# radoslawkrolikowski/financial-market-data-analysis

Measured on NVIDIA H100. Metric: sequences/sec (train step) biGRU h=256 seq=128 feat=64, higher is better.
Workload: dtype bf16x3 (fp32-class: split bf16 operand pairs on tensor cores, fp32 accumulate / state / gradients)

## Files before the change

### financial_market_data_analysis_b200/csrc/tc_hopper.cuh

```cuda
#pragma once
#include "common.cuh"
#include "kernels_f32.cuh"
#include <algorithm>
#include <map>
#include <mutex>
#include <cuda.h>
#include <cuda_bf16.h>

namespace htc {

typedef __nv_bfloat16 bf16_t;

__device__ __forceinline__ uint32_t smem_u32(const void* p) { return (uint32_t)__cvta_generic_to_shared(p); }

__device__ __forceinline__ void split_bf16(float x, bf16_t& hi, bf16_t& lo) {
    hi = __float2bfloat16(x);
    lo = __float2bfloat16(x - __bfloat162float(hi));
}

__device__ __forceinline__ void ldsm_x4(uint32_t addr, uint32_t (&r)[4]) {
    asm volatile("ldmatrix.sync.aligned.m8n8.x4.shared.b16 {%0, %1, %2, %3}, [%4];"
                 : "=r"(r[0]), "=r"(r[1]), "=r"(r[2]), "=r"(r[3]) : "r"(addr));
}
__device__ __forceinline__ void ldsm_x2(uint32_t addr, uint32_t (&r)[2]) {
// ... 28 lines not shown
}

constexpr int WG_BM = 128, WG_BN = 128, WG_BK = 64;
constexpr int WG_CBOX = 64 * 32 * 4;
__host__ __device__ constexpr int wg_cboxes(int ns) { return ns == 1 ? 4 : 2; }
__host__ __device__ constexpr int wg_smem_bytes(int ns, int stages) {
    return 1024 + stages * 2 * (ns == 1 ? 1 : 2) * WG_BM * WG_BK * 2 + 2 * wg_cboxes(ns) * WG_CBOX + 2 * stages * 8;
}

__global__ void tc_pack_kernel(const float* __restrict__ src, int64_t s_r, int64_t s_k, int64_t zsrc, int R, int K, int Rp, int Kp,
                               bf16_t* __restrict__ hi, bf16_t* __restrict__ lo) {
    __shared__ float tile[32][33];
    const int z = blockIdx.z, r0 = blockIdx.y * 32, k0 = blockIdx.x * 32;
    const float* a = src + z * zsrc;
    const bool kfast = s_k == 1;
    for (int j = threadIdx.y; j < 32; j += 8) {
        const int r = r0 + (kfast ? j : threadIdx.x), k = k0 + (kfast ? threadIdx.x : j);
        float v = 0.f;
        if (r < R && k < K) v = a[(int64_t)r * s_r + (int64_t)k * s_k];
        if (kfast) tile[j][threadIdx.x] = v; else tile[threadIdx.x][j] = v;
    }
    __syncthreads();
    for (int j = threadIdx.y; j < 32; j += 8) {
        const int r = r0 + j, k = k0 + threadIdx.x;
        const int64_t o = ((int64_t)z * Rp + r) * Kp + k;
        bf16_t h, l;
        split_bf16(tile[j][threadIdx.x], h, l);
        hi[o] = h;
        if (lo) lo[o] = l;
    }
}

__global__ void to_planes_kernel(const float* __restrict__ src, int64_t rows, int cols, int pitch, bf16_t* __restrict__ hi,
                                 bf16_t* __restrict__ lo) {
    const int64_t n = rows * cols;
    for (int64_t i = (int64_t)blockIdx.x * blockDim.x + threadIdx.x; i < n; i += (int64_t)gridDim.x * blockDim.x) {
        const int64_t r = i / cols, c = i % cols, o = r * pitch + c;
        bf16_t h, l;
        split_bf16(src[i], h, l);
        hi[o] = h;
        if (lo) lo[o] = l;
    }
}

__device__ __forceinline__ void mbar_init(uint64_t* bar, uint32_t count) {
    asm volatile("mbarrier.init.shared::cta.b64 [%0], %1;" ::"r"(smem_u32(bar)), "r"(count) : "memory");
}
__device__ __forceinline__ void mbar_arrive_expect_tx(uint64_t* bar, uint32_t bytes) {
    asm volatile("mbarrier.arrive.expect_tx.shared::cta.b64 _, [%0], %1;" ::"r"(smem_u32(bar)), "r"(bytes) : "memory");
}
__device__ __forceinline__ void mbar_arrive(uint64_t* bar) {
    asm volatile("mbarrier.arrive.shared::cta.b64 _, [%0];" ::"r"(smem_u32(bar)) : "memory");
}
__device__ __forceinline__ bool mbar_try_wait(uint64_t* bar, uint32_t parity) {
    uint32_t ok;
    asm volatile(
        "{\n\t.reg .pred p;\n\t"
        "mbarrier.try_wait.parity.shared::cta.b64 p, [%1], %2;\n\t"
        "selp.u32 %0, 1, 0, p;\n\t}" : "=r"(ok) : "r"(smem_u32(bar)), "r"(parity) : "memory");
    return ok != 0;
}
__device__ __forceinline__ bool mbar_try_wait_cluster(uint64_t* bar, uint32_t parity) {
    uint32_t ok;
    asm volatile(
        "{\n\t.reg .pred p;\n\t"
        "mbarrier.try_wait.parity.acquire.cluster.shared::cta.b64 p, [%1], %2;\n\t"
        "selp.u32 %0, 1, 0, p;\n\t}" : "=r"(ok) : "r"(smem_u32(bar)), "r"(parity) : "memory");
    return ok != 0;
}
template <bool CLUSTER = false>
__device__ __forceinline__ void mbar_wait(uint64_t* bar, uint32_t parity) {
    auto ready = [&] { return CLUSTER ? mbar_try_wait_cluster(bar, parity) : mbar_try_wait(bar, parity); };
    if (ready()) return;
    uint64_t t0, t;
    asm volatile("mov.u64 %0, %%globaltimer;" : "=l"(t0));
    for (uint32_t i = 0;; ++i) {
        if (ready()) return;
        if ((i & 1023u) == 1023u) {
            asm volatile("mov.u64 %0, %%globaltimer;" : "=l"(t));
            if (t - t0 > 5000000000ull) __trap();
        }
    }
}
__device__ __forceinline__ void bulk_copy_to_peer(uint32_t src, uint32_t bytes, uint64_t* bar, uint32_t cta) {
    asm volatile("cp.async.bulk.shared::cluster.shared::cta.mbarrier::complete_tx::bytes [%0], [%1], %2, [%3];"
                 ::"r"(mapa(src, cta)), "r"(src), "r"(bytes), "r"(mapa(smem_u32(bar), cta)) : "memory");
}
__device__ __forceinline__ void tma_load_3d(uint32_t dst, const CUtensorMap* m, uint64_t* bar, int c0, int c1, int c2) {
    asm volatile("cp.async.bulk.tensor.3d.shared::cluster.global.mbarrier::complete_tx::bytes [%0], [%1, {%3, %4, %5}], [%2];"
                 ::"r"(dst), "l"(reinterpret_cast<uint64_t>(m)), "r"(smem_u32(bar)), "r"(c0), "r"(c1), "r"(c2) : "memory");
}
__device__ __forceinline__ void tma_store_3d(const CUtensorMap* m, uint32_t src, int c0, int c1, int c2) {
    asm volatile("cp.async.bulk.tensor.3d.global.shared::cta.bulk_group [%0, {%2, %3, %4}], [%1];"
                 ::"l"(reinterpret_cast<uint64_t>(m)), "r"(src), "r"(c0), "r"(c1), "r"(c2) : "memory");
}
__device__ __forceinline__ void bulk_commit() { asm volatile("cp.async.bulk.commit_group;" ::: "memory"); }
template <int N>
__device__ __forceinline__ void bulk_wait_read() { asm volatile("cp.async.bulk.wait_group.read %0;" ::"n"(N) : "memory"); }
__device__ __forceinline__ void bulk_wait_all() { asm volatile("cp.async.bulk.wait_group 0;" ::: "memory"); }
__device__ __forceinline__ void named_sync(int id, int n) { asm volatile("bar.sync %0, %1;" ::"r"(id), "r"(n) : "memory"); }
__device__ __forceinline__ uint64_t wg_desc(uint32_t saddr, uint32_t lbo) {
    return (uint64_t)((saddr & 0x3FFFF) >> 4) | ((uint64_t)(lbo >> 4) << 16) | ((uint64_t)(1024 >> 4) << 32) | ((uint64_t)1 << 62);
}
template <int TA, int TB>
__device__ __forceinline__ void wgmma_m64n128k16(float (&d)[64], uint64_t da, uint64_t db) {
    asm volatile("wgmma.mma_async.sync.aligned.m64n128k16.f32.bf16.bf16 {%0, %1, %2, %3, %4, %5, %6, %7, %8, %9, %10, %11, %12, %13, %14, %15, %16, %17, %18, %19, %20, %21, %22, %23, %24, %25, %26, %27, %28, %29, %30, %31, %32, %33, %34, %35, %36, %37, %38, %39, %40, %41, %42, %43, %44, %45, %46, %47, %48, %49, %50, %51, %52, %53, %54, %55, %56, %57, %58, %59, %60, %61, %62, %63}, %64, %65, 1, 1, 1, %66, %67;"
                 : "+f"(d[0]), "+f"(d[1]), "+f"(d[2]), "+f"(d[3]), "+f"(d[4]), "+f"(d[5]), "+f"(d[6]), "+f"(d[7]), "+f"(d[8]), "+f"(d[9]), "+f"(d[10]), "+f"(d[11]), "+f"(d[12]), "+f"(d[13]), "+f"(d[14]), "+f"(d[15]), "+f"(d[16]), "+f"(d[17]), "+f"(d[18]), "+f"(d[19]), "+f"(d[20]), "+f"(d[21]), "+f"(d[22]), "+f"(d[23]), "+f"(d[24]), "+f"(d[25]), "+f"(d[26]), "+f"(d[27]), "+f"(d[28]), "+f"(d[29]), "+f"(d[30]), "+f"(d[31]), "+f"(d[32]), "+f"(d[33]), "+f"(d[34]), "+f"(d[35]), "+f"(d[36]), "+f"(d[37]), "+f"(d[38]), "+f"(d[39]), "+f"(d[40]), "+f"(d[41]), "+f"(d[42]), "+f"(d[43]), "+f"(d[44]), "+f"(d[45]), "+f"(d[46]), "+f"(d[47]), "+f"(d[48]), "+f"(d[49]), "+f"(d[50]), "+f"(d[51]), "+f"(d[52]), "+f"(d[53]), "+f"(d[54]), "+f"(d[55]), "+f"(d[56]), "+f"(d[57]), "+f"(d[58]), "+f"(d[59]), "+f"(d[60]), "+f"(d[61]), "+f"(d[62]), "+f"(d[63])
                 : "l"(da), "l"(db), "n"(TA), "n"(TB));
}

struct WgOp {
    int zsel, coff, kshift[2];
};
struct WgJob {
    WgOp a, b;
    float* C; const float* bias; float* part;
    int M, N, tm, tn, batch, splits;
    int kblocks, kbd;
    int kcat;
    int beta;
    int cmap;
    int64_t ldc, zC, zBias;
};

template <int NS, int STAGES, int AMN, int BMN>
__global__ void __launch_bounds__(384, 1)
wg_gemm_kernel(const __grid_constant__ CUtensorMap ta_hi, const __grid_constant__ CUtensorMap ta_lo,
               const __grid_constant__ CUtensorMap tb_hi, const __grid_constant__ CUtensorMap tb_lo,
               const __grid_constant__ CUtensorMap tc, const WgJob j) {
    constexpr int NH = NS == 1 ? 1 : 2;
    constexpr int PLANE = WG_BM * WG_BK * 2;
    constexpr int STAGE = 2 * NH * PLANE;
    constexpr int CB = wg_cboxes(NS);
    extern __shared__ __align__(1024) uint8_t wg_smem_raw[];
    uint8_t* sm = reinterpret_cast<uint8_t*>((reinterpret_cast<uintptr_t>(wg_smem_raw) + 1023) & ~(uintptr_t)1023);
    uint64_t* full = reinterpret_cast<uint64_t*>(sm + STAGES * STAGE + 2 * CB * WG_CBOX);
    uint64_t* empty = full + STAGES;
    const int wgi = threadIdx.x / 128, tid = threadIdx.x % 128;
    const int units = j.tm * j.tn * j.batch * j.splits;
    const int per = (j.kblocks + j.splits - 1) / j.splits;
    if (threadIdx.x == 0) {
        for (int i = 0; i < STAGES; ++i) { mbar_init(full + i, 1); mbar_init(empty + i, 2); }
        asm volatile("fence.mbarrier_init.release.cluster;" ::: "memory");
    }
    __syncthreads();
    auto decode = [&](int u, int& s, int& zb, int& m0, int& n0) {
        s = u % j.splits; u /= j.splits;
        n0 = (u % j.tn) * WG_BN; u /= j.tn;
        m0 = (u % j.tm) * WG_BM; zb = u / j.tm;
    };

    if (wgi == 0) {
        if (tid == 0) {
            uint32_t it = 0;
            for (int u = blockIdx.x; u < units; u += gridDim.x) {
                int s, zb, m0, n0;
                decode(u, s, zb, m0, n0);
                const int kb1 = min(j.kblocks, (s + 1) * per);
                for (int kb = s * per; kb < kb1; ++kb, ++it) {
                    const int st = it % STAGES;
                    if (it >= STAGES) mbar_wait(empty + st, ((it / STAGES) - 1) & 1);
                    const uint32_t base = smem_u32(sm + st * STAGE);
                    mbar_arrive_expect_tx(full + st, STAGE);
                    const int dz = j.kcat ? kb / j.kbd : zb, kc = (j.kcat ? kb % j.kbd : kb) * WG_BK;
#pragma unroll
                    for (int h = 0; h < NH; ++h) {
                        const CUtensorMap* ma = h ? &ta_lo : &ta_hi;
                        const CUtensorMap* mb = h ? &tb_lo : &tb_hi;
                        const uint32_t da = base + h * PLANE, db = base + (NH + h) * PLANE;
// ... 63 lines not shown
                for (int e = 0; e < 2; ++e) {
                    const int gn = n0 + 8 * i + 2 * q + e;
                    bv[2 * i + e] = bias && gn < j.N ? bias[gn] : 0.f;
                }
            uint8_t* stg = sm + STAGES * STAGE + cg * CB * WG_CBOX;
#pragma unroll
            for (int c = 0; c < 4; ++c) {
                const uint32_t box = smem_u32(stg + (c % CB) * WG_CBOX);
                if (tid == 0) bulk_wait_read<CB - 1>();
                named_sync(1 + cg, 128);
#pragma unroll
                for (int ii = 0; ii < 4; ++ii) {
                    const int i = 4 * c + ii;
#pragma unroll
                    for (int h = 0; h < 2; ++h) {
                        float v0 = d[4 * i + 2 * h], v1 = d[4 * i + 2 * h + 1];
                        if (bias) { v0 += bv[2 * i]; v1 += bv[2 * i + 1]; }
                        const uint32_t a = box + (w * 16 + r8 + 8 * h) * 128 + (((2 * ii + (q >> 1)) ^ r8) << 4) + (q & 1) * 8;
                        asm volatile("st.shared.v2.f32 [%0], {%1, %2};" ::"r"(a), "f"(v0), "f"(v1) : "memory");
                    }
                }
                asm volatile("fence.proxy.async.shared::cta;" ::: "memory");
                named_sync(1 + cg, 128);
                if (tid == 0) {
                    if (n0 + 32 * c < j.N) tma_store_3d(&tc, box, n0 + 32 * c, m0 + cg * 64, zc);
                    bulk_commit();
                }
            }
            continue;
        }
        float* C;
        int64_t ldc;
        const float* bias = nullptr;
        if (j.splits > 1) {
            C = j.part + ((int64_t)s * j.batch + zb) * j.M * j.N;
            ldc = j.N;
        } else {
            C = j.C + zb * j.zC;
            ldc = j.ldc;
            if (j.bias) bias = j.bias + zb * j.zBias;
        }
#pragma unroll
        for (int i = 0; i < 16; ++i)
#pragma unroll
            for (int e = 0; e < 4; ++e) {
                const int gm = m0 + cg * 64 + w * 16 + (l >> 2) + (e >= 2 ? 8 : 0);
                const int gn = n0 + 8 * i + 2 * (l & 3) + (e & 1);
                if (gm >= j.M || gn >= j.N) continue;
                float v = d[4 * i + e];
                if (bias) v += bias[gn];
                float* c = C + (int64_t)gm * ldc + gn;
                if (j.beta && j.splits == 1) *c += v;
                else *c = v;
            }
    }
    if (j.cmap && tid == 0) bulk_wait_all();
}

__global__ void splitk_reduce_kernel(const float* __restrict__ part, int splits, int batch, int M, int N, float* __restrict__ C,
                                     int64_t ldc, int64_t zC, int beta) {
    const int64_t per = (int64_t)M * N, n = per * batch;
    for (int64_t i = (int64_t)blockIdx.x * blockDim.x + threadIdx.x; i < n; i += (int64_t)gridDim.x * blockDim.x) {
        float v = 0.f;
        for (int s = 0; s < splits; ++s) v += part[(int64_t)s * n + i];
        const int64_t z = i / per, r = i % per;
        float* c = C + z * zC + (r / N) * ldc + r % N;
        *c = beta ? *c + v : v;
    }
}

constexpr int SCAN_U = 64, SCAN_NB = 16, SCAN_THREADS = 256;
constexpr int SCAN_Y = 1, SCAN_G = 2, SCAN_PLANES = 4;
constexpr int SCAN_TRAIN = SCAN_Y | SCAN_G | SCAN_PLANES, SCAN_INFER_LOWER = SCAN_PLANES, SCAN_INFER_TOP = SCAN_Y;

template <int H, int NS>
struct FwdSmem {
    static constexpr int NH = NS == 1 ? 1 : 2;
    static constexpr int NBMAX = NS == 1 ? SCAN_NB : 2 * SCAN_NB;
    static constexpr int NBUF = NBMAX == SCAN_NB ? 2 : 1;
    static constexpr int WP = H * 2;
    static constexpr int WBYTES = 3 * SCAN_U * WP;
    static constexpr int HBYTES = NBMAX * H * 2;
    static constexpr int SLICE = NBMAX * SCAN_U * 2;
    static constexpr int TOTAL = NH * WBYTES + NBUF * NH * HBYTES + 2 * 8;
};

__device__ __forceinline__ void scan_tile(int q, int m2, int ntd, int D, int& d, int& bt0, int& nb) {
    if (q < D * m2) {
        d = q / m2; bt0 = (q % m2) * 2 * SCAN_NB; nb = 2 * SCAN_NB;
    } else {
        const int r = q - D * m2, o = ntd - 2 * m2;
        d = r / o; bt0 = (2 * m2 + r % o) * SCAN_NB; nb = SCAN_NB;
    }
}

template <int NBMAX>
__device__ __forceinline__ uint32_t hsw(int b, int k) {
    return (uint32_t)((k / SCAN_U) * (NBMAX * SCAN_U * 2)) + swz<SCAN_U * 2>(b, k % SCAN_U);
}

__device__ __forceinline__ void mbar_arrive_peer(uint64_t* bar, uint32_t cta) {
    asm volatile("mbarrier.arrive.release.cluster.shared::cluster.b64 _, [%0];" ::"r"(mapa(smem_u32(bar), cta)) : "memory");
}

template <int H, int NS, int OUT, bool LEN, int JN, bool RD = false>
__device__ __forceinline__ void gru_scan_fwd_tile(const float* __restrict__ gi, const float* __restrict__ Whh,
                                                  const float* __restrict__ bhh, int64_t zW, const float* __restrict__ h0,
                                                  float* __restrict__ Y, float* __restrict__ G, float* __restrict__ hn_out,
                                                  bf16_t* __restrict__ yh, bf16_t* __restrict__ yl, int B, int T, int D,
                                                  const int* __restrict__ lens, int d, int bt0,
                                                  const float* __restrict__ mask = nullptr) {
    using S = FwdSmem<H, NS>;
    constexpr int U = SCAN_U, CS = H / U, NH = S::NH, JMAX = JN, jn = JN, nb = JN * SCAN_NB;
    constexpr int NBMAX = nb, NBUF = S::NBUF * S::NBMAX / nb;
    constexpr int HBYTES = nb * H * 2, SLICE = nb * U * 2;
    static_assert(NBUF * HBYTES == S::NBUF * S::HBYTES, "both tile sizes fill the h region");
    static_assert(SCAN_THREADS % (nb * (U / 8)) == 0, "a thread copies the same Y plane row in every pass");
    extern __shared__ __align__(128) uint8_t smem[];
    uint8_t* Wsm = smem;
    uint8_t* Hsm = smem + NH * S::WBYTES;
    uint64_t* full = reinterpret_cast<uint64_t*>(Hsm + NBUF * NH * HBYTES);
    uint64_t* empty = full + 1;
    const int c = (int)cluster_rank();
    const int tid = threadIdx.x, lane = tid & 31, warp = tid >> 5;
    const float* W = Whh + d * zW;

    for (int i = tid; i < 3 * U * H; i += SCAN_THREADS) {
        const int q = i / H, k = i % H, gte = q / U, u = q % U;
        const float v = W[(int64_t)(gte * H + c * U + u) * H + k];
        bf16_t hi, lo;
        split_bf16(v, hi, lo);
        *reinterpret_cast<bf16_t*>(Wsm + swz<S::WP>(q, k)) = hi;
        if (NH == 2) *reinterpret_cast<bf16_t*>(Wsm + S::WBYTES + swz<S::WP>(q, k)) = lo;
    }
    for (int i = tid; i < nb * H; i += SCAN_THREADS) {
        const int b = i / H, k = i % H;
        float v = h0 ? h0[((int64_t)d * B + bt0 + b) * H + k] : 0.f;
        if constexpr (RD) v *= mask[((int64_t)d * B + bt0 + b) * H + k];
        bf16_t hi, lo;
        split_bf16(v, hi, lo);
        *reinterpret_cast<bf16_t*>(Hsm + hsw<NBMAX>(b, k)) = hi;
        if (NH == 2) *reinterpret_cast<bf16_t*>(Hsm + HBYTES + hsw<NBMAX>(b, k)) = lo;
    }
    if (tid == 0) {
        mbar_init(full, 1);
        mbar_init(full + 1, NBUF == 2 ? 1 : CS - 1);
        asm volatile("fence.mbarrier_init.release.cluster;" ::: "memory");
    }

    const int ug = warp >> 1, nt = warp & 1;
    int unit[2], bcol[JMAX][2];
    unit[0] = ug * 16 + (lane >> 2); unit[1] = unit[0] + 8;
#pragma unroll
    for (int j = 0; j < JMAX; ++j) {
        bcol[j][0] = (nt * jn + j) * 8 + 2 * (lane & 3); bcol[j][1] = bcol[j][0] + 1;
    }
    float bias[3][2], hp[JMAX][4], mk[RD ? JMAX : 1][4];
#pragma unroll
    for (int gte = 0; gte < 3; ++gte)
#pragma unroll
        for (int i = 0; i < 2; ++i) bias[gte][i] = bhh[d * zW + gte * H + c * U + unit[i]];
    int len[JMAX][2], rlen = T;
#pragma unroll
    for (int j = 0; j < JMAX; ++j) {
#pragma unroll
        for (int e = 0; e < 4; ++e) {
            const int b = bt0 + bcol[j][e & 1], k = c * U + unit[e >> 1];
            hp[j][e] = h0 ? h0[((int64_t)d * B + b) * H + k] : 0.f;
            if constexpr (RD) mk[j][e] = mask[((int64_t)d * B + b) * H + k];
        }
        len[j][0] = len[j][1] = T;
        if (LEN) { len[j][0] = lens[bt0 + bcol[j][0]]; len[j][1] = lens[bt0 + bcol[j][1]]; }
    }
    if (LEN) rlen = lens[bt0 + (tid / (U / 8)) % nb];
    cluster_arrive();
    cluster_wait();

    const int DH = D * H;
    for (int s = 0; s < T; ++s) {
        const int t = d == 0 ? s : T - 1 - s;
        const int buf = NBUF == 2 ? s & 1 : 0, nbuf = NBUF == 2 ? buf ^ 1 : 0;
        if (s > 0) mbar_wait<true>(full + buf, (NBUF == 2 ? (s - 1) >> 1 : s - 1) & 1);
        if (tid == 0 && s + 1 < T) mbar_arrive_expect_tx(full + nbuf, (CS - 1) * NH * nb * U * 2);
        float giv[3][JMAX][4];
#pragma unroll
        for (int j = 0; j < JMAX; ++j)
#pragma unroll
            for (int e = 0; e < 4; ++e) {
                const int64_t row = (int64_t)(bt0 + bcol[j][e & 1]) * T + t;
                const float* gr = gi + ((int64_t)d * B * T + row) * 3 * H + c * U + unit[e >> 1];
#pragma unroll
                for (int gte = 0; gte < 3; ++gte) giv[gte][j][e] = gr[gte * H];
            }
        float acc[3][JMAX][4];
#pragma unroll
        for (int gte = 0; gte < 3; ++gte)
#pragma unroll
            for (int j = 0; j < JMAX; ++j)
#pragma unroll
                for (int e = 0; e < 4; ++e) acc[gte][j][e] = 0.f;
        const uint32_t hbase = smem_u32(Hsm + buf * NH * HBYTES);
        const uint32_t wbase = smem_u32(Wsm);
#pragma unroll 4
        for (int ks = 0; ks < H / 16; ++ks) {
            uint32_t bh[JMAX][NH][2];
            const int bk = ks * 16 + ((lane >> 3) & 1) * 8;
#pragma unroll
            for (int j = 0; j < JMAX; ++j)
#pragma unroll
                for (int h = 0; h < NH; ++h)
                    ldsm_x2(hbase + h * HBYTES + hsw<NBMAX>((nt * jn + j) * 8 + (lane & 7), bk), bh[j][h]);
#pragma unroll
            for (int gte = 0; gte < 3; ++gte) {
                const int arow = gte * U + ug * 16 + (lane & 15), ak = ks * 16 + (lane >> 4) * 8;
                uint32_t a[NH][4];
#pragma unroll
                for (int h = 0; h < NH; ++h) ldsm_x4(wbase + h * S::WBYTES + swz<S::WP>(arow, ak), a[h]);
#pragma unroll
                for (int j = 0; j < JMAX; ++j) {
                    if (NS != 1) {
                        mma_bf16(acc[gte][j], a[0], bh[j][NH - 1][0], bh[j][NH - 1][1]);
                        mma_bf16(acc[gte][j], a[NH - 1], bh[j][0][0], bh[j][0][1]);
                    }
                    mma_bf16(acc[gte][j], a[0], bh[j][0][0], bh[j][0][1]);
                }
            }
        }
        if (NBUF == 1) {
            __syncthreads();
            if (tid < CS - 1) mbar_arrive_peer(empty, (c + 1 + tid) % CS);
        }
        float hv[JMAX][4];
#pragma unroll
        for (int j = 0; j < JMAX; ++j)
#pragma unroll
            for (int e = 0; e < 4; ++e) {
                const int b = bt0 + bcol[j][e & 1], ul = unit[e >> 1], k = c * U + ul;
                const float r = sigmoid_f(giv[0][j][e] + acc[0][j][e] + bias[0][e >> 1]);
                const float z = sigmoid_f(giv[1][j][e] + acc[1][j][e] + bias[1][e >> 1]);
                const float hnv = acc[2][j][e] + bias[2][e >> 1];
                const float n = tanhf(giv[2][j][e] + r * hnv);
                const bool pad = LEN && t >= len[j][e & 1];
                float h;
                if constexpr (RD) h = pad ? hp[j][e] : (1.f - z) * n + z * (mk[j][e] * hp[j][e]);
                else h = pad ? hp[j][e] : (1.f - z) * n + z * hp[j][e];
                hp[j][e] = h;
                if constexpr (RD) hv[j][e] = mk[j][e] * h;
                else hv[j][e] = h;
                const int64_t row = (int64_t)b * T + t;
                if (OUT & SCAN_Y) Y[row * DH + d * H + k] = pad ? 0.f : h;
                if ((OUT & SCAN_G) && !pad) {
                    float* gs = G + ((int64_t)d * B * T + row) * 4 * H + k;
                    gs[0] = r; gs[H] = z; gs[2 * H] = n; gs[3 * H] = hnv;
                }
                if (hn_out && s == T - 1) hn_out[((int64_t)d * B + b) * H + k] = h;
            }
        if (NBUF == 1) mbar_wait<true>(empty, s & 1);
#pragma unroll
        for (int j = 0; j < JMAX; ++j)
#pragma unroll
            for (int e = 0; e < 4; ++e) {
                bf16_t hi, lo;
                split_bf16(hv[j][e], hi, lo);
                uint8_t* la = Hsm + nbuf * NH * HBYTES + hsw<NBMAX>(bcol[j][e & 1], c * U + unit[e >> 1]);
                *reinterpret_cast<bf16_t*>(la) = hi;
                if (NH == 2) *reinterpret_cast<bf16_t*>(la + HBYTES) = lo;
            }
        asm volatile("fence.proxy.async.shared::cta;" ::: "memory");
        __syncthreads();
        const uint32_t own = smem_u32(Hsm + nbuf * NH * HBYTES + c * SLICE);
        if (tid == 0 && s + 1 < T) {
#pragma unroll
            for (int p = 1; p < CS; ++p) {
                const uint32_t dst = (c + p) % CS;
#pragma unroll
                for (int h = 0; h < NH; ++h) bulk_copy_to_peer(own + h * HBYTES, nb * U * 2, full + nbuf, dst);
            }
        }
        if (OUT & SCAN_PLANES) {
            for (int i = tid; i < NH * nb * (U / 8); i += SCAN_THREADS) {
                const int h = i / (nb * U / 8), r = (i / (U / 8)) % nb, kl = (i % (U / 8)) * 8;
                uint4 v = *reinterpret_cast<const uint4*>(Hsm + (nbuf * NH + h) * HBYTES + c * SLICE + swz<U * 2>(r, kl));
                if (LEN && t >= rlen) v = make_uint4(0u, 0u, 0u, 0u);
                *reinterpret_cast<uint4*>((h ? yl : yh) + ((int64_t)(bt0 + r) * T + t) * DH + d * H + c * U + kl) = v;
            }
        }
    }
    cluster_arrive();
    cluster_wait();
}

template <int H, int NS, int OUT, bool LEN, bool RD>
__global__ void __launch_bounds__(SCAN_THREADS, 1)
gru_scan_fwd_kernel(const float* __restrict__ gi, const float* __restrict__ Whh, const float* __restrict__ bhh, int64_t zW,
                    const float* __restrict__ h0, float* __restrict__ Y, float* __restrict__ G, float* __restrict__ hn_out,
                    bf16_t* __restrict__ yh, bf16_t* __restrict__ yl, int B, int T, int D, int m2, const int* __restrict__ lens,
                    const float* __restrict__ mask) {
    static_assert(!RD || OUT == SCAN_TRAIN, "recurrent dropout runs in the training forward only");
    int d, bt0, nb;
    scan_tile(blockIdx.y, m2, B / SCAN_NB, D, d, bt0, nb);
    if constexpr (FwdSmem<H, NS>::NBMAX == 2 * SCAN_NB) {
        if (nb == 2 * SCAN_NB) {
            gru_scan_fwd_tile<H, NS, OUT, LEN, 2, RD>(gi, Whh, bhh, zW, h0, Y, G, hn_out, yh, yl, B, T, D, lens, d, bt0, mask);
            return;
        }
    }
    gru_scan_fwd_tile<H, NS, OUT, LEN, 1, RD>(gi, Whh, bhh, zW, h0, Y, G, hn_out, yh, yl, B, T, D, lens, d, bt0, mask);
}

template <int H, int NS>
struct BwdSmem {
    static constexpr int NH = NS == 1 ? 1 : 2;
    static constexpr int Q = 3 * SCAN_U;
    static constexpr int WP = Q * 2;
    static constexpr int WBYTES = H * WP;
    static constexpr int DBYTES = SCAN_NB * Q * 2;
    static constexpr int SLOT = SCAN_NB * SCAN_U * 4;
    static constexpr int TOTAL = NH * WBYTES + NH * DBYTES + (H / SCAN_U - 1) * SLOT;
    static_assert(NH * DBYTES >= SLOT, "own partial sums alias the dgh tile");
};

__device__ __forceinline__ int xslot(int kl, int b) {
    static_assert(SCAN_NB == 16, "eight column pairs per unit");
    const int g = ((kl >> 1) & 1) * 4 + ((kl >> 2) & 3);
    return kl * SCAN_NB + (((b >> 1) ^ g) << 1) + (b & 1);
}

template <int H, int NS, bool LEN, int NR, bool RD = false>
__device__ __forceinline__ void gru_scan_bwd_tile(const float* __restrict__ G, const float* __restrict__ Y,
                                                  const float* __restrict__ h0, const float* __restrict__ dY,
                                                  float* __restrict__ dhc, float* __restrict__ dgi, float* __restrict__ dgh,
                                                  const float* __restrict__ Whh, int64_t zW, bf16_t* __restrict__ gih,
                                                  bf16_t* __restrict__ gil, bf16_t* __restrict__ ghh, bf16_t* __restrict__ ghl,
                                                  int B, int T, int D, const int* __restrict__ lens, int d, int bt0,
                                                  const float* __restrict__ mask = nullptr) {
    using S = BwdSmem<H, NS>;
    constexpr int U = SCAN_U, CS = H / U, NH = S::NH, Q = S::Q, NB = SCAN_NB;
    constexpr int MT = H / 16 / 8;
    constexpr int PAIRS = NR * U / SCAN_THREADS;
    constexpr int NBLK = NR / 8;
    extern __shared__ __align__(128) uint8_t smem[];
    uint8_t* Wsm = smem;
    uint8_t* Dsm = smem + NH * S::WBYTES;
    float* recv = reinterpret_cast<float*>(Dsm + NH * S::DBYTES);
    const int c = (int)cluster_rank();
    const int tid = threadIdx.x, lane = tid & 31, warp = tid >> 5;
    const float* W = Whh + d * zW;
    float* own = reinterpret_cast<float*>(Dsm);
    auto slot = [&](int src) -> float* { return src == c ? own : recv + (src < c ? src : src - 1) * NB * U; };

    for (int i = tid; i < Q * H; i += SCAN_THREADS) {
        const int q = i / H, k = i % H, gte = q / U, u = q % U;
        const float v = W[(int64_t)(gte * H + c * U + u) * H + k];
        bf16_t hi, lo;
        split_bf16(v, hi, lo);
        *reinterpret_cast<bf16_t*>(Wsm + swz<S::WP>(k, q)) = hi;
        if (NH == 2) *reinterpret_cast<bf16_t*>(Wsm + S::WBYTES + swz<S::WP>(k, q)) = lo;
    }
    float dhr[PAIRS], dhz[PAIRS], mk[RD ? PAIRS : 1];
    int plen[PAIRS];
#pragma unroll
    for (int i = 0; i < PAIRS; ++i) {
        const int p = tid + i * SCAN_THREADS, u = p % U, b = p / U;
        dhr[i] = dhc[((int64_t)d * B + bt0 + b) * H + c * U + u];
        dhz[i] = 0.f;
        plen[i] = LEN ? lens[bt0 + b] : T;
        if constexpr (RD) mk[i] = mask[((int64_t)d * B + bt0 + b) * H + c * U + u];
    }
    cluster_arrive();
    cluster_wait();

    const int DH = D * H;
    float gr[PAIRS], gz[PAIRS], gn[PAIRS], ghn[PAIRS], hprev[PAIRS], dyv[PAIRS];
    auto load_step = [&](int s) {
        const int t = d == 0 ? T - 1 - s : s;
        const bool first = d == 0 ? t == 0 : t == T - 1;
#pragma unroll
        for (int i = 0; i < PAIRS; ++i) {
            const int p = tid + i * SCAN_THREADS, u = p % U, b = bt0 + p / U, j = c * U + u;
            const int64_t row = (int64_t)b * T + t;
            const float* gs = G + ((int64_t)d * B * T + row) * 4 * H + j;
            gr[i] = gs[0]; gz[i] = gs[H]; gn[i] = gs[2 * H]; ghn[i] = gs[3 * H];
            if (first) hprev[i] = h0 ? h0[((int64_t)d * B + b) * H + j] : 0.f;
            else hprev[i] = Y[((int64_t)b * T + (d == 0 ? t - 1 : t + 1)) * DH + d * H + j];
            dyv[i] = dY[row * DH + d * H + j];
            if constexpr (RD) hprev[i] *= mk[i];
        }
    };
    load_step(0);
    for (int s = 0; s < T; ++s) {
        const int t = d == 0 ? T - 1 - s : s;
        const bool first = d == 0 ? t == 0 : t == T - 1;
        if (s > 0) {
#pragma unroll
            for (int i = 0; i < PAIRS; ++i) {
                const int p = tid + i * SCAN_THREADS, x = xslot(p % U, p / U);
                float v = dhz[i];
#pragma unroll
                for (int src = 0; src < CS; ++src) v += slot(src)[x];
                if constexpr (RD) v = LEN && (d == 0 ? t + 1 : t - 1) >= plen[i] ? v : mk[i] * v;
                dhr[i] = v;
            }
        }
        cluster_arrive();
        __syncthreads();
#pragma unroll
        for (int i = 0; i < PAIRS; ++i) {
            const int p = tid + i * SCAN_THREADS, u = p % U, bl = p / U, b = bt0 + bl, j = c * U + u;
            const int64_t row = (int64_t)b * T + t;
            const float r = gr[i], z = gz[i], n = gn[i], hnv = ghn[i], hpv = hprev[i];
            const float dh = dhr[i] + dyv[i];
            float dan = dh * (1.f - z) * (1.f - n * n);
            float dar = dan * hnv * r * (1.f - r);
            float daz = dh * (hpv - n) * z * (1.f - z);
            float dgn = dan * r;
            const bool pad = LEN && t >= plen[i];
            if (pad) dan = dar = daz = dgn = 0.f;
            float* a = dgi + ((int64_t)d * B * T + row) * 3 * H + j;
            float* cg = dgh + ((int64_t)d * B * T + row) * 3 * H + j;
            a[0] = dar; a[H] = daz; a[2 * H] = dan;
            cg[0] = dar; cg[H] = daz; cg[2 * H] = dgn;
            dhz[i] = pad ? dhr[i] : dh * z;
            const float gv[3] = {dar, daz, dgn};
#pragma unroll
            for (int gte = 0; gte < 3; ++gte) {
                bf16_t hi, lo;
                split_bf16(gv[gte], hi, lo);
                *reinterpret_cast<bf16_t*>(Dsm + swz<S::WP>(bl, gte * U + u)) = hi;
                if (NH == 2) *reinterpret_cast<bf16_t*>(Dsm + S::DBYTES + swz<S::WP>(bl, gte * U + u)) = lo;
            }
            bf16_t hi, lo;
            split_bf16(dan, hi, lo);
            const int64_t po = ((int64_t)d * B * T + row) * 3 * H + 2 * H + j;
            gih[po] = hi;
            if (NH == 2) gil[po] = lo;
        }
        if (NS == 1 && s + 1 < T) load_step(s + 1);
        __syncthreads();
        for (int i = tid; i < NH * NR * (Q / 8); i += SCAN_THREADS) {
            const int h = i / (NR * Q / 8), r = (i / (Q / 8)) % NR, q = (i % (Q / 8)) * 8, gte = q / U;
            uint4 v = *reinterpret_cast<const uint4*>(Dsm + h * S::DBYTES + swz<S::WP>(r, q));
            const int64_t o = ((int64_t)d * B * T + (int64_t)(bt0 + r) * T + t) * 3 * H + gte * H + c * U + q % U;
            if (gte < 2) *reinterpret_cast<uint4*>((h ? gil : gih) + o) = v;
            if (first) v = make_uint4(0u, 0u, 0u, 0u);
            *reinterpret_cast<uint4*>((h ? ghl : ghh) + o) = v;
        }
        float acc[MT][2][4];
#pragma unroll
        for (int m = 0; m < MT; ++m)
#pragma unroll
            for (int n = 0; n < NBLK; ++n)
#pragma unroll
                for (int e = 0; e < 4; ++e) acc[m][n][e] = 0.f;
        const uint32_t wbase = smem_u32(Wsm), dbase = smem_u32(Dsm);
#pragma unroll 2
        for (int ks = 0; ks < Q / 16; ++ks) {
            uint32_t bv[NH][4];
            const int brow = (lane & 7) + ((lane >> 4) << 3), bk = ks * 16 + ((lane >> 3) & 1) * 8;
#pragma unroll
            for (int h = 0; h < NH; ++h) ldsm_x4(dbase + h * S::DBYTES + swz<S::WP>(brow, bk), bv[h]);
#pragma unroll
            for (int m = 0; m < MT; ++m) {
                const int arow = (warp + 8 * m) * 16 + (lane & 15), ak = ks * 16 + (lane >> 4) * 8;
                uint32_t a[NH][4];
#pragma unroll
                for (int h = 0; h < NH; ++h) ldsm_x4(wbase + h * S::WBYTES + swz<S::WP>(arow, ak), a[h]);
#pragma unroll
                for (int n = 0; n < NBLK; ++n) {
                    if (NS != 1) {
                        mma_bf16(acc[m][n], a[0], bv[NH - 1][2 * n], bv[NH - 1][2 * n + 1]);
                        mma_bf16(acc[m][n], a[NH - 1], bv[0][2 * n], bv[0][2 * n + 1]);
                    }
                    mma_bf16(acc[m][n], a[0], bv[0][2 * n], bv[0][2 * n + 1]);
                }
            }
        }
        if (NS != 1 && s + 1 < T) load_step(s + 1);
        __syncthreads();
        cluster_wait();
#pragma unroll
        for (int m = 0; m < MT; ++m)
#pragma unroll
            for (int n = 0; n < NBLK; ++n)
#pragma unroll
                for (int e = 0; e < 4; e += 2) {
                    const int k = (warp + 8 * m) * 16 + (lane >> 2) + (e >= 2 ? 8 : 0);
                    const int bl = n * 8 + 2 * (lane & 3);
                    const int dst = k / U, x = xslot(k % U, bl);
                    const float2 v = make_float2(acc[m][n][e], acc[m][n][e + 1]);
                    if (dst == c) {
                        *reinterpret_cast<float2*>(own + x) = v;
                    } else {
                        const float* rs = recv + (c < dst ? c : c - 1) * NB * U + x;
                        st_cluster_v2_f32(mapa(smem_u32(rs), dst), v);
                    }
                }
        cluster_arrive();
        cluster_wait();
    }
#pragma unroll
    for (int i = 0; i < PAIRS; ++i) {
        const int p = tid + i * SCAN_THREADS, u = p % U, b = p / U, x = xslot(u, b);
        float v = dhz[i];
#pragma unroll
        for (int src = 0; src < CS; ++src) v += slot(src)[x];
        if constexpr (RD) v = LEN && (d == 0 ? 0 : T - 1) >= plen[i] ? v : mk[i] * v;
        dhc[((int64_t)d * B + bt0 + b) * H + c * U + u] = v;
    }
}

template <int H, int NS, bool LEN, bool RD>
__global__ void __launch_bounds__(SCAN_THREADS, 1)
gru_scan_bwd_kernel(const float* __restrict__ G, const float* __restrict__ Y, const float* __restrict__ h0,
                    const float* __restrict__ dY, float* __restrict__ dhc, float* __restrict__ dgi, float* __restrict__ dgh,
                    const float* __restrict__ Whh, int64_t zW, bf16_t* __restrict__ gih, bf16_t* __restrict__ gil,
                    bf16_t* __restrict__ ghh, bf16_t* __restrict__ ghl, int B, int T, int D, int L8, const int* __restrict__ lens,
                    const float* __restrict__ mask) {
    const int ntd = B / SCAN_NB, n16 = D * ntd - L8, q = blockIdx.y;
    if (q < n16) {
        gru_scan_bwd_tile<H, NS, LEN, SCAN_NB, RD>(G, Y, h0, dY, dhc, dgi, dgh, Whh, zW, gih, gil, ghh, ghl, B, T, D, lens,
                                                    q / ntd, (q % ntd) * SCAN_NB, mask);
    } else {
        const int f = n16 + (q - n16) / 2;
        gru_scan_bwd_tile<H, NS, LEN, SCAN_NB / 2, RD>(G, Y, h0, dY, dhc, dgi, dgh, Whh, zW, gih, gil, ghh, ghl, B, T, D, lens,
                                                        f / ntd, (f % ntd) * SCAN_NB + ((q - n16) & 1) * (SCAN_NB / 2), mask);
    }
}

}

static inline int64_t rup(int64_t v, int64_t m) { return (v + m - 1) / m * m; }
static inline int64_t tc_pack_elems(int64_t R, int64_t K, int64_t batch, int prec) {
    return (prec == BIGRU_PREC_BF16X3 ? 2 : 1) * batch * rup(R, htc::WG_BM) * rup(K, htc::WG_BK);
}
static inline int64_t tc_gemm_ws_elems(int64_t M, int64_t N, int64_t K, int64_t batch, int prec) {
    return tc_pack_elems(M, K, batch, prec) + tc_pack_elems(N, K, batch, prec);
}
static inline int wg_splits(int64_t tiles, int64_t kblocks) {
    const int64_t s = std::min(cdiv64(4 * 132, tiles), kblocks / 8);
    if (s <= 1) return 1;
    const int64_t per = cdiv64(kblocks, s);
    return (int)cdiv64(kblocks, per);
}

struct Planes {
    const htc::bf16_t* hi; const htc::bf16_t* lo;
    int64_t cols, rows, depth, pitch;
};

typedef CUresult (*PFN_encodeTiled_t)(CUtensorMap*, CUtensorMapDataType, cuuint32_t, void*, const cuuint64_t*, const cuuint64_t*,
                                      const cuuint32_t*, const cuuint32_t*, CUtensorMapInterleave, CUtensorMapSwizzle,
                                      CUtensorMapL2promotion, CUtensorMapFloatOOBfill);
static int encode_map(CUtensorMap* m, CUtensorMapDataType type, int esize, const void* base, int64_t cols, int64_t rows,
                      int64_t depth, int64_t pitch, int64_t zstride, uint32_t box0, uint32_t box1) {
    static PFN_encodeTiled_t enc = nullptr;
    if (!enc) {
        void* f = nullptr;
        cudaDriverEntryPointQueryResult q;
        if (cudaGetDriverEntryPoint("cuTensorMapEncodeTiled", &f, cudaEnableDefault, &q) != cudaSuccess || q != cudaDriverEntryPointSuccess) {
            bigru_set_error("tc_gemm: cuTensorMapEncodeTiled is unavailable");
            return BIGRU_ERR_CUDA;
        }
        enc = (PFN_encodeTiled_t)f;
    }
    const cuuint64_t dims[3] = {(cuuint64_t)cols, (cuuint64_t)rows, (cuuint64_t)depth};
    const cuuint64_t strides[2] = {(cuuint64_t)(pitch * esize), (cuuint64_t)(zstride * esize)};
    const cuuint32_t box[3] = {box0, box1, 1u}, es[3] = {1u, 1u, 1u};
    CUresult r = enc(m, type, 3, const_cast<void*>(base), dims, strides, box, es, CU_TENSOR_MAP_INTERLEAVE_NONE,
                     CU_TENSOR_MAP_SWIZZLE_128B, CU_TENSOR_MAP_L2_PROMOTION_L2_256B, CU_TENSOR_MAP_FLOAT_OOB_FILL_NONE);
    if (r != CUDA_SUCCESS) { bigru_set_error("tc_gemm: cuTensorMapEncodeTiled failed (%d)", (int)r); return BIGRU_ERR_CUDA; }
    return BIGRU_OK;
}

static int make_plane_map(CUtensorMap* m, const htc::bf16_t* base, const Planes& p, bool mn) {
    return encode_map(m, CU_TENSOR_MAP_DATA_TYPE_BFLOAT16, 2, base, p.cols, p.rows, p.depth, p.pitch, p.pitch * p.rows, 64u,
                      mn ? 64u : 128u);
}

template <int NS, int AMN, int BMN>
static int wg_launch(const CUtensorMap (&tm)[5], const htc::WgJob& j, int grid, cudaStream_t st) {
    constexpr int STAGES = NS == 1 ? 4 : 3;
    constexpr int smem = htc::wg_smem_bytes(NS, STAGES);
    static_assert(smem <= 232448, "wg_gemm_kernel: more shared memory than an sm_90 block may have");
    auto k = htc::wg_gemm_kernel<NS, STAGES, AMN, BMN>;
    CUDA_TRY(cudaFuncSetAttribute(k, cudaFuncAttributeMaxDynamicSharedMemorySize, smem));
    k<<<grid, 384, smem, st>>>(tm[0], tm[1], tm[2], tm[3], tm[4], j);
    LAUNCH_CHECK();
    return BIGRU_OK;
}

// ... 252 lines not shown
```

Measured before the change: 52040.

## Prefetch next-step gate inputs and add a single-warp-group bf16 scan multiply

The forward GRU scan now loads the next time step's input-gate values (gi) at the end of each step, so the global-load latency overlaps the bulk copies and plane stores instead of sitting on the critical path. For the pure bf16 (NS==1) variant, only four warps run the recurrent multiply: they cover all batch columns with software-pipelined fragment loads, then hand half of the accumulators to the other warps through shared memory using named barriers. That variant also gets an extra shared-memory exchange area and a 2-blocks-per-SM launch bound. Prefetching keeps the gi values live across the MMA loop, which raises register pressure.

Measured after the change: 52250, median of 6. No clear change (+0.4%).

```diff
diff --git a/financial_market_data_analysis_b200/csrc/tc_hopper.cuh b/financial_market_data_analysis_b200/csrc/tc_hopper.cuh
--- a/financial_market_data_analysis_b200/csrc/tc_hopper.cuh
+++ b/financial_market_data_analysis_b200/csrc/tc_hopper.cuh
@@ -366,7 +366,9 @@
     static constexpr int WBYTES = 3 * SCAN_U * WP;
     static constexpr int HBYTES = NBMAX * H * 2;
     static constexpr int SLICE = NBMAX * SCAN_U * 2;
-    static constexpr int TOTAL = NH * WBYTES + NBUF * NH * HBYTES + 2 * 8;
+    static constexpr int PEER = H / SCAN_U - 1;
+    static constexpr int XBYTES = NS == 1 && PEER < 3 ? (3 - PEER) * SLICE : 0;
+    static constexpr int TOTAL = NH * WBYTES + NBUF * NH * HBYTES + XBYTES + 2 * 8;
 };
 
 __device__ __forceinline__ void scan_tile(int q, int m2, int ntd, int D, int& d, int& bt0, int& nb) {
@@ -403,7 +405,8 @@
     extern __shared__ __align__(128) uint8_t smem[];
     uint8_t* Wsm = smem;
     uint8_t* Hsm = smem + NH * S::WBYTES;
-    uint64_t* full = reinterpret_cast<uint64_t*>(Hsm + NBUF * NH * HBYTES);
+    uint8_t* Xsm = Hsm + NBUF * NH * HBYTES;
+    uint64_t* full = reinterpret_cast<uint64_t*>(Xsm + S::XBYTES);
     uint64_t* empty = full + 1;
     const int c = (int)cluster_rank();
     const int tid = threadIdx.x, lane = tid & 31, warp = tid >> 5;
@@ -432,7 +435,8 @@
         asm volatile("fence.mbarrier_init.release.cluster;" ::: "memory");
     }
 
-    const int ug = warp >> 1, nt = warp & 1;
+    constexpr bool ONCE = NS == 1;
+    const int ug = ONCE ? warp & 3 : warp >> 1, nt = ONCE ? warp >> 2 : warp & 1;
     int unit[2], bcol[JMAX][2];
     unit[0] = ug * 16 + (lane >> 2); unit[1] = unit[0] + 8;
 #pragma unroll
@@ -461,58 +465,112 @@
     cluster_wait();
 
     const int DH = D * H;
+    float giv[3][JMAX][4];
+    auto load_gi = [&](int t) {
+#pragma unroll
+        for (int j = 0; j < JMAX; ++j)
+#pragma unroll
+            for (int e = 0; e < 4; ++e) {
+                const int64_t row = (int64_t)(bt0 + bcol[j][e & 1]) * T + t;
+                const float* gr = gi + ((int64_t)d * B * T + row) * 3 * H + c * U + unit[e >> 1];
+#pragma unroll
+                for (int gte = 0; gte < 3; ++gte) giv[gte][j][e] = gr[gte * H];
+            }
+    };
+    load_gi(d == 0 ? 0 : T - 1);
     for (int s = 0; s < T; ++s) {
         const int t = d == 0 ? s : T - 1 - s;
         const int buf = NBUF == 2 ? s & 1 : 0, nbuf = NBUF == 2 ? buf ^ 1 : 0;
         if (s > 0) mbar_wait<true>(full + buf, (NBUF == 2 ? (s - 1) >> 1 : s - 1) & 1);
         if (tid == 0 && s + 1 < T) mbar_arrive_expect_tx(full + nbuf, (CS - 1) * NH * nb * U * 2);
-        float giv[3][JMAX][4];
-#pragma unroll
-        for (int j = 0; j < JMAX; ++j)
-#pragma unroll
-            for (int e = 0; e < 4; ++e) {
-                const int64_t row = (int64_t)(bt0 + bcol[j][e & 1]) * T + t;
-                const float* gr = gi + ((int64_t)d * B * T + row) * 3 * H + c * U + unit[e >> 1];
-#pragma unroll
-                for (int gte = 0; gte < 3; ++gte) giv[gte][j][e] = gr[gte * H];
-            }
-        float acc[3][JMAX][4];
+        float acc[3][ONCE ? 2 * JN : JN][4];
 #pragma unroll
         for (int gte = 0; gte < 3; ++gte)
 #pragma unroll
-            for (int j = 0; j < JMAX; ++j)
+            for (int j = 0; j < (ONCE ? 2 * JN : JN); ++j)
 #pragma unroll
                 for (int e = 0; e < 4; ++e) acc[gte][j][e] = 0.f;
         const uint32_t hbase = smem_u32(Hsm + buf * NH * HBYTES);
         const uint32_t wbase = smem_u32(Wsm);
+        if constexpr (ONCE) {
+            static_assert(!ONCE || (NH == 1 && NBUF == 2), "the W-once multiply is the bf16 16-row one");
+            constexpr int NB8 = 2 * JN, KS = H / 16;
+            if (warp < 4) {
+                auto frag = [&](int ks, uint32_t (&fa)[3][4], uint32_t (&fb)[NB8][2]) {
+                    const int bk = ks * 16 + ((lane >> 3) & 1) * 8, ak = ks * 16 + (lane >> 4) * 8;
+#pragma unroll
+                    for (int j = 0; j < NB8; ++j) ldsm_x2(hbase + hsw<NBMAX>(j * 8 + (lane & 7), bk), fb[j]);
+#pragma unroll
+                    for (int gte = 0; gte < 3; ++gte) ldsm_x4(wbase + swz<S::WP>(gte * U + ug * 16 + (lane & 15), ak), fa[gte]);
+                };
+                auto mul = [&](const uint32_t (&fa)[3][4], const uint32_t (&fb)[NB8][2]) {
+#pragma unroll
+                    for (int gte = 0; gte < 3; ++gte)
+#pragma unroll
+                        for (int j = 0; j < NB8; ++j) mma_bf16(acc[gte][j], fa[gte], fb[j][0], fb[j][1]);
+                };
+                uint32_t a[2][3][4], bh[2][NB8][2];
+                frag(0, a[0], bh[0]);
+#pragma unroll 2
+                for (int ks = 0; ks < KS; ks += 2) {
+                    frag(ks + 1, a[1], bh[1]);
+                    mul(a[0], bh[0]);
+                    if (ks + 2 < KS) frag(ks + 2, a[0], bh[0]);
+                    mul(a[1], bh[1]);
+                }
+            }
+            auto slot = [&](int g) -> uint8_t* {
+                return g < S::PEER ? Hsm + buf * HBYTES + (c + 1 + g) % CS * SLICE : Xsm + (g - S::PEER) * SLICE;
+            };
+            if (warp < 4) {
+                named_sync(1, 128);
+#pragma unroll
+                for (int gte = 0; gte < 3; ++gte)
+#pragma unroll
+                    for (int j = 0; j < JN; ++j)
+                        *reinterpret_cast<float4*>(slot(gte) + (j * 128 + tid) * 16) =
+                            make_float4(acc[gte][JN + j][0], acc[gte][JN + j][1], acc[gte][JN + j][2], acc[gte][JN + j][3]);
+            }
+            named_sync(2 + ug, 64);
+            if (warp >= 4) {
+#pragma unroll
+                for (int gte = 0; gte < 3; ++gte)
+#pragma unroll
+                    for (int j = 0; j < JN; ++j) {
+                        const float4 v = *reinterpret_cast<const float4*>(slot(gte) + (j * 128 + tid - 128) * 16);
+                        acc[gte][j][0] = v.x; acc[gte][j][1] = v.y; acc[gte][j][2] = v.z; acc[gte][j][3] = v.w;
+                    }
+            }
+        } else {
 #pragma unroll 4
-        for (int ks = 0; ks < H / 16; ++ks) {
-            uint32_t bh[JMAX][NH][2];
-            const int bk = ks * 16 + ((lane >> 3) & 1) * 8;
-#pragma unroll
-            for (int j = 0; j < JMAX; ++j)
-#pragma unroll
-                for (int h = 0; h < NH; ++h)
-                    ldsm_x2(hbase + h * HBYTES + hsw<NBMAX>((nt * jn + j) * 8 + (lane & 7), bk), bh[j][h]);
-#pragma unroll
-            for (int gte = 0; gte < 3; ++gte) {
-                const int arow = gte * U + ug * 16 + (lane & 15), ak = ks * 16 + (lane >> 4) * 8;
-                uint32_t a[NH][4];
-#pragma unroll
-                for (int h = 0; h < NH; ++h) ldsm_x4(wbase + h * S::WBYTES + swz<S::WP>(arow, ak), a[h]);
-#pragma unroll
-                for (int j = 0; j < JMAX; ++j) {
-                    if (NS != 1) {
-                        mma_bf16(acc[gte][j], a[0], bh[j][NH - 1][0], bh[j][NH - 1][1]);
-                        mma_bf16(acc[gte][j], a[NH - 1], bh[j][0][0], bh[j][0][1]);
+            for (int ks = 0; ks < H / 16; ++ks) {
+                uint32_t bh[JMAX][NH][2];
+                const int bk = ks * 16 + ((lane >> 3) & 1) * 8;
+#pragma unroll
+                for (int j = 0; j < JMAX; ++j)
+#pragma unroll
+                    for (int h = 0; h < NH; ++h)
+                        ldsm_x2(hbase + h * HBYTES + hsw<NBMAX>((nt * jn + j) * 8 + (lane & 7), bk), bh[j][h]);
+#pragma unroll
+                for (int gte = 0; gte < 3; ++gte) {
+                    const int arow = gte * U + ug * 16 + (lane & 15), ak = ks * 16 + (lane >> 4) * 8;
+                    uint32_t a[NH][4];
+#pragma unroll
+                    for (int h = 0; h < NH; ++h) ldsm_x4(wbase + h * S::WBYTES + swz<S::WP>(arow, ak), a[h]);
+#pragma unroll
+                    for (int j = 0; j < JMAX; ++j) {
+                        if (NS != 1) {
+                            mma_bf16(acc[gte][j], a[0], bh[j][NH - 1][0], bh[j][NH - 1][1]);
+                            mma_bf16(acc[gte][j], a[NH - 1], bh[j][0][0], bh[j][0][1]);
+                        }
+                        mma_bf16(acc[gte][j], a[0], bh[j][0][0], bh[j][0][1]);
                     }
-                    mma_bf16(acc[gte][j], a[0], bh[j][0][0], bh[j][0][1]);
                 }
             }
-        }
-        if (NBUF == 1) {
-            __syncthreads();
-            if (tid < CS - 1) mbar_arrive_peer(empty, (c + 1 + tid) % CS);
+            if (NBUF == 1) {
+                __syncthreads();
+                if (tid < CS - 1) mbar_arrive_peer(empty, (c + 1 + tid) % CS);
+            }
         }
         float hv[JMAX][4];
 #pragma unroll
@@ -561,6 +619,7 @@
                 for (int h = 0; h < NH; ++h) bulk_copy_to_peer(own + h * HBYTES, nb * U * 2, full + nbuf, dst);
             }
         }
+        if (s + 1 < T) load_gi(d == 0 ? s + 1 : T - 2 - s);
         if (OUT & SCAN_PLANES) {
             for (int i = tid; i < NH * nb * (U / 8); i += SCAN_THREADS) {
                 const int h = i / (nb * U / 8), r = (i / (U / 8)) % nb, kl = (i % (U / 8)) * 8;
@@ -575,7 +634,7 @@
 }
 
 template <int H, int NS, int OUT, bool LEN, bool RD>
-__global__ void __launch_bounds__(SCAN_THREADS, 1)
+__global__ void __launch_bounds__(SCAN_THREADS, NS == 1 && H <= 256 ? 2 : 1)
 gru_scan_fwd_kernel(const float* __restrict__ gi, const float* __restrict__ Whh, const float* __restrict__ bhh, int64_t zW,
                     const float* __restrict__ h0, float* __restrict__ Y, float* __restrict__ G, float* __restrict__ hn_out,
                     bf16_t* __restrict__ yh, bf16_t* __restrict__ yl, int B, int T, int D, int m2, const int* __restrict__ lens,
```

## Exchange backward-scan partial sums via bulk copies and mbarriers instead of cluster barriers

Applied to the files above, without the earlier changes.

For H<=256 the backward GRU scan now writes each peer's partial sums into local staging slots. One thread pushes them to peers with cp.async.bulk, and full/empty mbarriers replace the two cluster-wide barriers per timestep. The staging writes for the next step's dgh tile are deferred until peers signal their receive buffers are free, and the next-step load is issued earlier. The aim is to cut per-step cluster synchronisation and DSMEM store latency, at the cost of more shared memory and more complex parity-based handshakes.

Result: faster. 52330 before, 53970 after (median of 6 runs) (+3.1%).

```diff
diff --git a/financial_market_data_analysis_b200/csrc/tc_hopper.cuh b/financial_market_data_analysis_b200/csrc/tc_hopper.cuh
--- a/financial_market_data_analysis_b200/csrc/tc_hopper.cuh
+++ b/financial_market_data_analysis_b200/csrc/tc_hopper.cuh
@@ -134,9 +134,12 @@
         }
     }
 }
+__device__ __forceinline__ void bulk_copy_to_peer_at(uint32_t dst, uint32_t src, uint32_t bytes, uint64_t* bar, uint32_t cta) {
+    asm volatile("cp.async.bulk.shared::cluster.shared::cta.mbarrier::complete_tx::bytes [%0], [%1], %2, [%3];"
+                 ::"r"(mapa(dst, cta)), "r"(src), "r"(bytes), "r"(mapa(smem_u32(bar), cta)) : "memory");
+}
 __device__ __forceinline__ void bulk_copy_to_peer(uint32_t src, uint32_t bytes, uint64_t* bar, uint32_t cta) {
-    asm volatile("cp.async.bulk.shared::cluster.shared::cta.mbarrier::complete_tx::bytes [%0], [%1], %2, [%3];"
-                 ::"r"(mapa(src, cta)), "r"(src), "r"(bytes), "r"(mapa(smem_u32(bar), cta)) : "memory");
+    bulk_copy_to_peer_at(src, src, bytes, bar, cta);
 }
 __device__ __forceinline__ void tma_load_3d(uint32_t dst, const CUtensorMap* m, uint64_t* bar, int c0, int c1, int c2) {
     asm volatile("cp.async.bulk.tensor.3d.shared::cluster.global.mbarrier::complete_tx::bytes [%0], [%1, {%3, %4, %5}], [%2];"
@@ -595,13 +598,17 @@
 template <int H, int NS>
 struct BwdSmem {
     static constexpr int NH = NS == 1 ? 1 : 2;
+    static constexpr int CS = H / SCAN_U;
     static constexpr int Q = 3 * SCAN_U;
     static constexpr int WP = Q * 2;
     static constexpr int WBYTES = H * WP;
     static constexpr int DBYTES = SCAN_NB * Q * 2;
     static constexpr int SLOT = SCAN_NB * SCAN_U * 4;
-    static constexpr int TOTAL = NH * WBYTES + NH * DBYTES + (H / SCAN_U - 1) * SLOT;
+    static constexpr bool BULK = H <= 256;
+    static constexpr int XBYTES = BULK && CS * SLOT > NH * DBYTES ? CS * SLOT : NH * DBYTES;
+    static constexpr int TOTAL = NH * WBYTES + XBYTES + (CS - 1) * SLOT + (BULK ? 2 * 8 : 0);
     static_assert(NH * DBYTES >= SLOT, "own partial sums alias the dgh tile");
+    static_assert(TOTAL <= 232448, "an H100 block's shared memory");
 };
 
 __device__ __forceinline__ int xslot(int kl, int b) {
@@ -626,11 +633,13 @@
     extern __shared__ __align__(128) uint8_t smem[];
     uint8_t* Wsm = smem;
     uint8_t* Dsm = smem + NH * S::WBYTES;
-    float* recv = reinterpret_cast<float*>(Dsm + NH * S::DBYTES);
+    float* recv = reinterpret_cast<float*>(Dsm + S::XBYTES);
+    uint64_t* full = reinterpret_cast<uint64_t*>(recv + (CS - 1) * NB * U);
+    uint64_t* empty = full + 1;
     const int c = (int)cluster_rank();
     const int tid = threadIdx.x, lane = tid & 31, warp = tid >> 5;
     const float* W = Whh + d * zW;
-    float* own = reinterpret_cast<float*>(Dsm);
+    float* own = reinterpret_cast<float*>(Dsm + (S::BULK ? c * S::SLOT : 0));
     auto slot = [&](int src) -> float* { return src == c ? own : recv + (src < c ? src : src - 1) * NB * U; };
 
     for (int i = tid; i < Q * H; i += SCAN_THREADS) {
@@ -650,6 +659,12 @@
         dhz[i] = 0.f;
         plen[i] = LEN ? lens[bt0 + b] : T;
         if constexpr (RD) mk[i] = mask[((int64_t)d * B + bt0 + b) * H + c * U + u];
+    }
+    if (S::BULK && tid == 0) {
+        mbar_init(full, 1);
+        mbar_init(empty, CS - 1);
+        asm volatile("fence.mbarrier_init.release.cluster;" ::: "memory");
+        mbar_arrive_expect_tx(full, (CS - 1) * S::SLOT);
     }
     cluster_arrive();
     cluster_wait();
@@ -676,6 +691,10 @@
         const int t = d == 0 ? T - 1 - s : s;
         const bool first = d == 0 ? t == 0 : t == T - 1;
         if (s > 0) {
+            if constexpr (S::BULK) {
+                mbar_wait<true>(full, (s - 1) & 1);
+                if (tid == 0) mbar_arrive_expect_tx(full, (CS - 1) * S::SLOT);
+            }
 #pragma unroll
             for (int i = 0; i < PAIRS; ++i) {
                 const int p = tid + i * SCAN_THREADS, x = xslot(p % U, p / U);
@@ -686,8 +705,10 @@
                 dhr[i] = v;
             }
         }
-        cluster_arrive();
+        if constexpr (!S::BULK) cluster_arrive();
         __syncthreads();
+        if (S::BULK && s > 0 && tid < CS - 1) mbar_arrive_peer(empty, (c + 1 + tid) % CS);
+        float gv[PAIRS][3];
 #pragma unroll
         for (int i = 0; i < PAIRS; ++i) {
             const int p = tid + i * SCAN_THREADS, u = p % U, bl = p / U, b = bt0 + bl, j = c * U + u;
@@ -705,21 +726,26 @@
             a[0] = dar; a[H] = daz; a[2 * H] = dan;
             cg[0] = dar; cg[H] = daz; cg[2 * H] = dgn;
             dhz[i] = pad ? dhr[i] : dh * z;
-            const float gv[3] = {dar, daz, dgn};
-#pragma unroll
-            for (int gte = 0; gte < 3; ++gte) {
-                bf16_t hi, lo;
-                split_bf16(gv[gte], hi, lo);
-                *reinterpret_cast<bf16_t*>(Dsm + swz<S::WP>(bl, gte * U + u)) = hi;
-                if (NH == 2) *reinterpret_cast<bf16_t*>(Dsm + S::DBYTES + swz<S::WP>(bl, gte * U + u)) = lo;
-            }
+            gv[i][0] = dar; gv[i][1] = daz; gv[i][2] = dgn;
             bf16_t hi, lo;
             split_bf16(dan, hi, lo);
             const int64_t po = ((int64_t)d * B * T + row) * 3 * H + 2 * H + j;
             gih[po] = hi;
             if (NH == 2) gil[po] = lo;
         }
-        if (NS == 1 && s + 1 < T) load_step(s + 1);
+        if (S::BULK && s > 0) mbar_wait<true>(empty, (s - 1) & 1);
+#pragma unroll
+        for (int i = 0; i < PAIRS; ++i) {
+            const int p = tid + i * SCAN_THREADS, u = p % U, bl = p / U;
+#pragma unroll
+            for (int gte = 0; gte < 3; ++gte) {
+                bf16_t hi, lo;
+                split_bf16(gv[i][gte], hi, lo);
+                *reinterpret_cast<bf16_t*>(Dsm + swz<S::WP>(bl, gte * U + u)) = hi;
+                if (NH == 2) *reinterpret_cast<bf16_t*>(Dsm + S::DBYTES + swz<S::WP>(bl, gte * U + u)) = lo;
+            }
+        }
+        if (s + 1 < T) load_step(s + 1);
         __syncthreads();
         for (int i = tid; i < NH * NR * (Q / 8); i += SCAN_THREADS) {
             const int h = i / (NR * Q / 8), r = (i / (Q / 8)) % NR, q = (i % (Q / 8)) * 8, gte = q / U;
@@ -759,9 +785,8 @@
                 }
             }
         }
-        if (NS != 1 && s + 1 < T) load_step(s + 1);
         __syncthreads();
-        cluster_wait();
+        if constexpr (!S::BULK) cluster_wait();
 #pragma unroll
         for (int m = 0; m < MT; ++m)
 #pragma unroll
@@ -772,16 +797,32 @@
                     const int bl = n * 8 + 2 * (lane & 3);
                     const int dst = k / U, x = xslot(k % U, bl);
                     const float2 v = make_float2(acc[m][n][e], acc[m][n][e + 1]);
-                    if (dst == c) {
+                    if (S::BULK) {
+                        *reinterpret_cast<float2*>(Dsm + dst * S::SLOT + x * 4) = v;
+                    } else if (dst == c) {
                         *reinterpret_cast<float2*>(own + x) = v;
                     } else {
                         const float* rs = recv + (c < dst ? c : c - 1) * NB * U + x;
                         st_cluster_v2_f32(mapa(smem_u32(rs), dst), v);
                     }
                 }
-        cluster_arrive();
-        cluster_wait();
-    }
+        if constexpr (S::BULK) {
+            asm volatile("fence.proxy.async.shared::cta;" ::: "memory");
+            __syncthreads();
+            if (tid == 0) {
+#pragma unroll
+                for (int p = 1; p < CS; ++p) {
+                    const int dst = (c + p) % CS;
+                    bulk_copy_to_peer_at(smem_u32(recv + (c < dst ? c : c - 1) * NB * U), smem_u32(Dsm + dst * S::SLOT),
+                                         S::SLOT, full, dst);
+                }
+            }
+        } else {
+            cluster_arrive();
+            cluster_wait();
+        }
+    }
+    if constexpr (S::BULK) mbar_wait<true>(full, (T - 1) & 1);
 #pragma unroll
     for (int i = 0; i < PAIRS; ++i) {
         const int p = tid + i * SCAN_THREADS, u = p % U, b = p / U, x = xslot(u, b);
@@ -790,6 +831,10 @@
         for (int src = 0; src < CS; ++src) v += slot(src)[x];
         if constexpr (RD) v = LEN && (d == 0 ? 0 : T - 1) >= plen[i] ? v : mk[i] * v;
         dhc[((int64_t)d * B + bt0 + b) * H + c * U + u] = v;
+    }
+    if constexpr (S::BULK) {
+        cluster_arrive();
+        cluster_wait();
     }
 }
 
```
